# benfred/implicit

Hardware: AMD Instinct MI355X
Metric: ALS user+item updates/sec per iteration (factors=128); top-k recs/sec (higher is better)
Workload: dtype f32; 1 GPU; BASELINE configs[2]: last.fm-360K-shaped synthetic CSR, ALS CG cg_steps=3; users=358868, items=292385, nnz=17308340, factors=128, solver=cg, cg_steps=3

## Files before the change

implicit_amd/csrc/als_cg_q.hip:

```cpp
#include <type_traits>

#include "als_qtile.h"
#include "common.h"

namespace imp {

template <typename T>
void launch_team_fused(const imp_csr *C, int f, int width, int first, int count, T *X, const T *Y, const float *A0, int cg_steps,
                       const char *name);
template <typename T>
void launch_group_fused(const imp_csr *C, int f, int first, int count, T *X, const T *Y, const float *A0, int cg_steps, const char *name);
template <typename ST>
void launch_team_tile64(const imp_csr *C, int f, int width, int first, int count, ST *X, const ST *Y, const float *A0, int cg_steps,
                        const char *name);

template <typename T>
void launch_team_chain(const imp_csr *C, int f, const int (&first)[3], const int (&count)[3], T *X, const T *Y, const float *A0, int cg_steps,
                       const char *name);

template <int F, typename T> static void run_classes_q(const imp_csr *C, T *X, const T *Y, const float *A0, int cg_steps) {
  const int32_t *b = C->bin_start;
  constexpr bool kHalf = std::is_same<T, __half>::value;
  auto team = [&](int width32, int lo, int hi, const char *name) {
    if constexpr (kHalf) launch_team_tile64<T>(C, F, width32 / 2, lo, hi - lo, X, Y, A0, cg_steps, name);
    else launch_team_fused<T>(C, F, width32, lo, hi - lo, X, Y, A0, cg_steps, name);
  };
  team(16, b[1], b[2], "als_cg_team16_rows");
  if (F == 128 && !kHalf && !prof_unfiltered()) {
    const int first[3] = {b[2], b[3], b[4]}, count[3] = {b[3] - b[2], b[4] - b[3], b[5] - b[4]};
    launch_team_chain<T>(C, F, first, count, X, Y, A0, cg_steps, "als_cg_team_chain_rows");
  } else {
    team(8, b[2], b[3], "als_cg_team8_rows");
    team(4, b[3], b[4], "als_cg_team4_rows");
    team(2, b[4], b[5], "als_cg_team2_rows");
  }
  if constexpr (F == 64) launch_team_fused<T>(C, F, 1, b[5], b[7] - b[5], X, Y, A0, cg_steps, "als_cg_short_rows");
  else launch_group_fused<T>(C, F, b[5], b[7] - b[5], X, Y, A0, cg_steps, "als_cg_short_rows");
}

template <typename T> void least_squares_cg_q(const imp_csr *C, T *X, const T *Y, const float *A0, int f, int cg_steps) {
  if (f == 128) run_classes_q<128, T>(C, X, Y, A0, cg_steps);
  else if (f == 64) run_classes_q<64, T>(C, X, Y, A0, cg_steps);
  else throw std::invalid_argument("least_squares_cg_q: f must be 64 or 128");
}
template void least_squares_cg_q<float>(const imp_csr *, float *, const float *, const float *, int, int);
template void least_squares_cg_q<__half>(const imp_csr *, __half *, const __half *, const float *, int, int);

}
```

implicit_amd/csrc/als_cg_qf.hip:

```cpp
#include <type_traits>

#include <algorithm>

#include "als_qf_common.h"
#include "common.h"

namespace imp {

template <typename ST> struct Tile32 {
  typedef f32x2 elem;
  static constexpr int T = 32;
  static constexpr bool ROLL = std::is_same<ST, float>::value;
  static __device__ __forceinline__ void fetch(const int32_t *indices, const float *data, int lane, int k0, int end, int &col, float &c) {
    fetch_entries(indices, data, lane, k0, end, col, c);
  }
  template <int H> static __device__ __forceinline__ void gather(elem (&yq)[H], const ST *p) {
#pragma unroll
    for (int h = 0; h < H; h += 2) {
      const float4 v = load4(p + 32 * h);
      yq[h] = f32x2{v.x, v.y}, yq[h + 1] = f32x2{v.z, v.w};
    }
  }
  template <int H> static __device__ __forceinline__ float dot(const elem (&yq)[H], const f32x2 (&ve)[H]) {
    f32x2 s = yq[0] * ve[0];
// ... 156 lines not shown
  auto axpy = [&](int q, float w) { Tile::template axpy<H>(y[q], w, ae); };
  static_for<4>([&](auto Pc) {
    constexpr int P = decltype(Pc)::value;
    if (8 * P < cnt) {
      const float cm1_0 = cwg[8 * P];
      float cm1_1 = 0.f, cp_0 = 0.f, cp_1 = 0.f;
      if constexpr (!LAST) cm1_1 = cwg[8 * P + 4];
      if constexpr (FIRST) cp_0 = cwg[32 + 8 * P], cp_1 = cwg[32 + 8 * P + 4];
      const float u = reduce_pair(partial(2 * P), partial(2 * P + 1));
      if constexpr (LAST) {
        s8 = fmaf(cm1_0 * u, u, s8);
      } else {
        const float w0 = FIRST ? fmaf(-cm1_0, row_bcast_from<0>(u), cp_0) : cm1_0 * row_bcast_from<0>(u);
        const float w1 = FIRST ? fmaf(-cm1_1, row_bcast_from<8>(u), cp_1) : cm1_1 * row_bcast_from<8>(u);
        axpy(2 * P, w0);
        axpy(2 * P + 1, w1);
      }
    }
    if constexpr (ROLL) {
      if (8 * P < cnt_nx) gather_pair<Tile, F, P>(y, cw, col_nx, c_nx, cnt_nx, Y, lane);
    }
  });
  if constexpr (LAST) {
    return 0.125f * s8;
  } else {
    float aes[FE];
#pragma unroll
    for (int h = 0; h < H; ++h) aes[2 * h] = ae[h].x, aes[2 * h + 1] = ae[h].y;
    reduce_expanded<F>(aes, acc);
    return 0.f;
  }
}

template <int F, typename ST>
__global__ __launch_bounds__(1024) void als_cg_qfgroup_kernel(const int32_t *__restrict__ order, int first, int count,
                                                              const int32_t *__restrict__ indptr,
                                                              const int32_t *__restrict__ indices,
                                                              const float *__restrict__ data, ST *__restrict__ X,
                                                              const ST *__restrict__ Y, const float *__restrict__ A0, int cg_steps) {
  using Cfg = QFGroupCfg<F>;
  constexpr int FC = F / 64, FE = F / 16, LD = Cfg::LD;
  constexpr bool ROLL = Tile32<ST>::ROLL;
  extern __shared__ __attribute__((aligned(16))) float smem[];
  constexpr int LDB = Cfg::LDB;
  __bf16 *A0b = reinterpret_cast<__bf16 *>(smem);
  __bf16 *Pb = A0b + (size_t)3 * F * LDB;
  float *Ps = reinterpret_cast<float *>(Pb + (size_t)3 * 16 * LDB);
  float *Outs = Ps + 16 * LD;
  float *cws = Outs + (size_t)Cfg::KH * 16 * LD;
  const int lane = threadIdx.x & 63;
  const int wave = __builtin_amdgcn_readfirstlane(threadIdx.x >> 6);
  for (int e = threadIdx.x; e < F * F; e += 1024) {
    int r = e / F, c = e - r * F;
    __bf16 h, m, l;
    split_bf16(A0[e], h, m, l);
    A0b[r * LDB + c] = h, A0b[(size_t)F * LDB + r * LDB + c] = m, A0b[(size_t)2 * F * LDB + r * LDB + c] = l;
  }
  __syncthreads();
  float *prow = Ps + (size_t)wave * LD;
  float *cw = cws + (size_t)wave * 64;
  const unsigned cf = (unsigned)QL<F>::cfactor(lane, 0);

  auto publish = [&](const float (&vec)[FC], bool valid) {
    if constexpr (FC == 2) *reinterpret_cast<float2 *>(prow + cf) = valid ? make_float2(vec[0], vec[1]) : make_float2(0.f, 0.f);
    else prow[cf] = valid ? vec[0] : 0.f;
    bf16x2 t[3];
#pragma unroll
    for (int c = 0; c < 2; ++c) {
      __bf16 h, m, l;
      split_bf16(valid ? vec[c] : 0.f, h, m, l);
      t[0][c] = h, t[1][c] = m, t[2][c] = l;
    }
#pragma unroll
    for (int k = 0; k < 3; ++k) *reinterpret_cast<bf16x2 *>(Pb + (size_t)k * 16 * LDB + (size_t)wave * LDB + cf) = t[k];
    __syncthreads();
  };
  auto product = [&]() {
    const int ti = wave % Cfg::NT, kh = wave / Cfg::NT;
    const int ln = opaque(lane);
    const int i = ln & 15, kq = ln >> 4;
    f32x4 acc = {0.f, 0.f, 0.f, 0.f};
    static_assert(Cfg::KB * 16 == 64, "three-term product: 64 k per wave");
#pragma unroll
    for (int b = 0; b < 2; ++b) {
      const int k0 = kh * 64 + 32 * b + 8 * kq;
      const __bf16 *ar = A0b + (size_t)(16 * ti + i) * LDB + k0, *pr = Pb + (size_t)i * LDB + k0;
      const bf16x8 ah = *reinterpret_cast<const bf16x8 *>(ar), am = *reinterpret_cast<const bf16x8 *>(ar + (size_t)F * LDB),
                   al = *reinterpret_cast<const bf16x8 *>(ar + (size_t)2 * F * LDB);
      const bf16x8 ph = *reinterpret_cast<const bf16x8 *>(pr), pm = *reinterpret_cast<const bf16x8 *>(pr + (size_t)16 * LDB),
                   pl = *reinterpret_cast<const bf16x8 *>(pr + (size_t)2 * 16 * LDB);
      acc = __builtin_amdgcn_mfma_f32_16x16x32_bf16(al, ph, acc, 0, 0, 0);
      acc = __builtin_amdgcn_mfma_f32_16x16x32_bf16(ah, pl, acc, 0, 0, 0);
      acc = __builtin_amdgcn_mfma_f32_16x16x32_bf16(am, pm, acc, 0, 0, 0);
      acc = __builtin_amdgcn_mfma_f32_16x16x32_bf16(am, ph, acc, 0, 0, 0);
      acc = __builtin_amdgcn_mfma_f32_16x16x32_bf16(ah, pm, acc, 0, 0, 0);
      acc = __builtin_amdgcn_mfma_f32_16x16x32_bf16(ah, ph, acc, 0, 0, 0);
    }
    *reinterpret_cast<float4 *>(Outs + (kh * 16 + i) * LD + 16 * ti + 4 * kq) = make_float4(acc[0], acc[1], acc[2], acc[3]);
  };
  auto collect = [&](float (&out)[FC]) {
#pragma unroll
    for (int c = 0; c < FC; ++c) out[c] = 0.f;
#pragma unroll
    for (int h = 0; h < Cfg::KH; ++h) {
      const float *o = Outs + (h * 16 + wave) * LD + cf;
      if constexpr (FC == 2) {
        const float2 t = *reinterpret_cast<const float2 *>(o);
        out[0] += t.x, out[1] += t.y;
      } else {
        out[0] += o[0];
      }
    }
  };
  const bool product_first = ((wave >> 2) & 1) == 0;

  const int groups = (count + 15) / 16, g_step = gridDim.x;
  auto row_id = [&](int g) { return order[first + min(g * 16 + wave, count - 1)]; };
  auto row_valid = [&](int g) { return g < groups && g * 16 + wave < count; };
  int id0 = row_id(blockIdx.x), id1 = row_id(blockIdx.x + g_step), id2 = row_id(blockIdx.x + 2 * g_step), id3 = row_id(blockIdx.x + 3 * g_step);
  int b0 = indptr[id0], e0 = indptr[id0 + 1], b1 = indptr[id1], e1 = indptr[id1 + 1], b2 = indptr[id2], e2 = indptr[id2 + 1];
  int ent_col, ent_cnt = row_valid(blockIdx.x) ? e0 - b0 : 0;
  float ent_c;
  fetch_entries(indices, data, opaque(lane), b0, max(e0, b0 + 1), ent_col, ent_c);
  bool tile_ready = false;
  int cnt = 0;
  f32x2 y[8][FE / 2];
  float x[FC];
  auto kill = [](float (&v)[FC]) {
#pragma unroll
    for (int cc = 0; cc < FC; ++cc) v[cc] = 0.f;
  };
  kill(x);
  for (int g = blockIdx.x; g < groups; g += g_step) {
    const bool valid = row_valid(g);
    ST *xrow = X + (size_t)id0 * F;
    if (!tile_ready) {
      cnt = ent_cnt;
      ent_col = opaque(ent_col);
      ent_c = __int_as_float(opaque(__float_as_int(ent_c)));
      static_for<4>([&](auto Pc) {
        constexpr int P = decltype(Pc)::value;
        if (8 * P < cnt) gather_pair<Tile32<ST>, F, P>(y, cw, ent_col, ent_c, cnt, Y, lane);
      });
      ent_cnt = row_valid(g + g_step) ? e1 - b1 : 0;
      fetch_entries(indices, data, opaque(lane), b1, max(e1, b1 + 1), ent_col, ent_c);
      load_compact<F>(xrow, opaque(lane), x);
    }
    float xc[FC], r[FC], p[FC], Ap[FC], sp[FC];
#pragma unroll
    for (int cc = 0; cc < FC; ++cc) xc[cc] = x[cc];
    publish(xc, valid);
    if (!product_first) tile_pass<F, true, false, false, ST>(y, cw, cnt, prow, sp, lane, 0, ent_col, ent_c, Y);
    product();
    if (product_first) tile_pass<F, true, false, false, ST>(y, cw, cnt, prow, sp, lane, 0, ent_col, ent_c, Y);
    __syncthreads();
    collect(Ap);
#pragma unroll
    for (int cc = 0; cc < FC; ++cc) p[cc] = r[cc] = sp[cc] - Ap[cc];
    float rsold = dot_compact<F>(r, r);
    bool active = valid && rsold >= 1e-20f;
    const bool store = active;
    for (int it = 0; it + 1 < cg_steps; ++it) {
      publish(p, active);
      if (active && !product_first) tile_pass<F, false, false, false, ST>(y, cw, cnt, prow, sp, lane, 0, ent_col, ent_c, Y);
      product();
      if (active && product_first) tile_pass<F, false, false, false, ST>(y, cw, cnt, prow, sp, lane, 0, ent_col, ent_c, Y);
      __syncthreads();
      collect(Ap);
      if (active) {
#pragma unroll
        for (int cc = 0; cc < FC; ++cc) Ap[cc] += sp[cc];
        const float alpha = rsold * __builtin_amdgcn_rcpf(dot_compact<F>(p, Ap));
#pragma unroll
        for (int cc = 0; cc < FC; ++cc) {
          xc[cc] = fmaf(alpha, p[cc], xc[cc]);
          r[cc] = fmaf(-alpha, Ap[cc], r[cc]);
        }
        const float rsnew = dot_compact<F>(r, r);
        if (rsnew < 1e-20f) {
          active = false;
        } else {
          const float beta = rsnew * __builtin_amdgcn_rcpf(rsold);
#pragma unroll
          for (int cc = 0; cc < FC; ++cc) p[cc] = fmaf(beta, p[cc], r[cc]);
          rsold = rsnew;
        }
      }
    }
    bool rolled = false;
    if (cg_steps > 0) {
      publish(p, active);
      float tile_pAp = 0.f;
      auto last_tiles = [&]() {
        if constexpr (ROLL) tile_pAp = tile_pass<F, false, true, true, ST>(y, cw, cnt, prow, sp, lane, ent_cnt, ent_col, ent_c, Y);
        else tile_pAp = tile_pass<F, false, true, false, ST>(y, cw, cnt, prow, sp, lane, 0, ent_col, ent_c, Y);
      };
      if (active && !product_first) last_tiles();
      product();
      if (active && product_first) last_tiles();
      __syncthreads();
      collect(Ap);
      if (active) {
        if constexpr (ROLL) {
          cnt = ent_cnt;
          ent_cnt = row_valid(g + 2 * g_step) ? e2 - b2 : 0;
          fetch_entries(indices, data, opaque(lane), b2, max(e2, b2 + 1), ent_col, ent_c);
          load_compact<F>(X + (size_t)id1 * F, opaque(lane), x);
          rolled = true;
        } else {
          kill(x);
        }
        const float alpha = rsold * __builtin_amdgcn_rcpf(wave_allsum(dot_local<FC>(p, Ap) + tile_pAp));
#pragma unroll
        for (int cc = 0; cc < FC; ++cc) xc[cc] = fmaf(alpha, p[cc], xc[cc]);
      } else {
        kill(x);
      }
    } else {
      kill(x);
    }
    if (store) store_compact<F>(xrow, opaque(lane), xc);
    tile_ready = rolled;
    id0 = id1, id1 = id2, id2 = id3, id3 = row_id(g + 4 * g_step);
    b0 = b1, e0 = e1, b1 = b2, e1 = e2, b2 = indptr[id2], e2 = indptr[id2 + 1];
  }
}

template <typename T>
static void launch_qfgroup(const imp_csr *C, int first, int count, T *X, const T *Y, const float *A0, int cg_steps, const char *name) {
  if (count <= 0) return;
  constexpr int F = 128;
  const size_t lds = QFGroupCfg<F>::lds_bytes;
  auto kern = als_cg_qfgroup_kernel<F, T>;
  IMP_CHECK_HIP(hipFuncSetAttribute(reinterpret_cast<const void *>(kern), hipFuncAttributeMaxDynamicSharedMemorySize, (int)lds));
  int grid = std::min((count + 15) / 16, ctx().num_cus * std::max(2, ctx().oversub));
  IMP_PROF(name);
  kern<<<grid, 1024, lds, stream()>>>(C->order.data(), first, count, C->indptr.data(), C->indices.data(), C->data.data(), X, Y, A0,
                                      cg_steps);
  IMP_CHECK_HIP(hipGetLastError());
}

template <typename T>
void launch_group_fused(const imp_csr *C, int f, int first, int count, T *X, const T *Y, const float *A0, int cg_steps, const char *name) {
  if (f == 128) launch_qfgroup<T>(C, first, count, X, Y, A0, cg_steps, name);
  else throw std::invalid_argument("launch_group_fused: f must be 128 (f = 64 short rows run on independent wavefronts)");
}
template void launch_group_fused<float>(const imp_csr *, int, int, int, float *, const float *, const float *, int, const char *);
template void launch_group_fused<__half>(const imp_csr *, int, int, int, __half *, const __half *, const float *, int, const char *);

template <typename T>
void launch_team_fused(const imp_csr *C, int f, int width, int first, int count, T *X, const T *Y, const float *A0, int cg_steps,
                       const char *name) {
  if constexpr (std::is_same<T, __half>::value) {
    if (f != 64 || width != 1) throw std::invalid_argument("launch_team_fused: float16 storage takes the f = 64 short rows only");
    launch_qfteam<64, 1, 512, T>(C, first, count, X, Y, A0, cg_steps, name);
  } else {
    auto run = [&](auto Fc) {
      constexpr int F = decltype(Fc)::value;
      switch (width) {
        case 16: launch_qfteam<F, 16, 1024, T>(C, first, count, X, Y, A0, cg_steps, name); break;
        case 8: launch_qfteam<F, 8, 512, T>(C, first, count, X, Y, A0, cg_steps, name); break;
        case 4: launch_qfteam<F, 4, 512, T>(C, first, count, X, Y, A0, cg_steps, name); break;
        case 2: launch_qfteam<F, 2, 512, T>(C, first, count, X, Y, A0, cg_steps, name); break;
        case 1:
          if constexpr (F == 64) launch_qfteam<F, 1, 512, T>(C, first, count, X, Y, A0, cg_steps, name);
          else throw std::invalid_argument("launch_team_fused: one wave per row needs f = 64");
          break;
        default: throw std::invalid_argument("launch_team_fused: team width");
      }
    };
    if (f == 128) run(idx_t<128>{});
    else if (f == 64) run(idx_t<64>{});
    else throw std::invalid_argument("launch_team_fused: f must be 64 or 128");
// ... 8 lines not shown
```

implicit_amd/csrc/common.h:

```cpp
#ifndef IMPLICIT_AMD_CSRC_COMMON_H_
#define IMPLICIT_AMD_CSRC_COMMON_H_

#include <hip/hip_runtime.h>

#include <climits>
#include <cstdint>
#include <cstdio>
#include <memory>
#include <mutex>
#include <optional>
#include <stdexcept>
#include <string>
#include <vector>

#include "../../include/implicit_hip.h"
#include "csr_schedule.h"
#include "team_tickets.h"

namespace imp {

struct out_of_range_error : std::runtime_error {
  using std::runtime_error::runtime_error;
};

// ... 122 lines not shown
    const char *a = static_cast<const char *>(dst), *b = static_cast<const char *>(y_src);
    return b && a < b + y_rows * (size_t)y_f * sizeof(float) && b < a + bytes;
  }
  void release() {
    x = {}, y = {}, gram = {};
    forget_y();
  }
};

struct Context {
  int device = 0;
  hipStream_t stream = nullptr;
  int num_cus = 256;
  int oversub = 1;
  bool deferred = false;
  hipStream_t occupy_stream = nullptr;
  std::recursive_mutex mutex;
  std::mutex small_mutex;
  std::vector<void *> small_free[24];
  void *pin_stage = nullptr;
  size_t pin_stage_bytes = 0;
  hipEvent_t pin_stage_ev = nullptr;
  DeviceArray<float> gram_ws;
  DeviceArray<float> long_ws;
  PaddedSystem pad;
  DeviceArray<double> loss_buf;
  DeviceArray<unsigned long long> chol_failed;
  DeviceArray<float> barrier_word;
  unsigned long long *fixup_total = nullptr;
  DeviceArray<float> w256_ws;
  DeviceArray<unsigned> nm_fix_rows;
  DeviceArray<unsigned> chain_counters;
  ChainTickets chain_tickets;
  DeviceArray<int> nm_ticket;
  DeviceArray<unsigned long long> bpr_stats;
  DeviceArray<float> lmf_ws;
  DeviceArray<double> knn_acc;
  DeviceArray<int32_t> knn_touched;
  int knn_cols = -1;
};
inline hipStream_t stream() { return ctx().stream; }
void note_device_write(const void *dst, size_t bytes);
struct DerivedCache {
  const void *src = nullptr;
  size_t bytes = 0;
};
void register_derived_cache(DerivedCache *c);
void unregister_derived_cache(DerivedCache *c);

}

struct imp_matrix {
  size_t rows = 0, cols = 0, itemsize = 4;
  void *data = nullptr;
  std::shared_ptr<imp::Storage> storage;
  size_t bytes() const { return rows * cols * itemsize; }
  float *f32() const {
    if (itemsize != 4) throw std::runtime_error("can't cast Matrix to float*");
    return reinterpret_cast<float *>(data);
  }
};

struct imp_intvector {
  imp::DeviceArray<int32_t> v;
  size_t size = 0;
};
// ... 76 lines not shown
```

implicit_amd/csrc/containers.hip:

```cpp
#include <hip/hip_fp16.h>

#include <algorithm>
#include <cstring>
#include <map>
#include <mutex>
#include <thread>

#include "common.h"

namespace imp {

static thread_local std::string g_last_error;
void set_last_error(const std::string &msg) { g_last_error = msg; }

static std::mutex g_ctx_mutex;
static auto &g_contexts = *new std::map<int, std::unique_ptr<Context>>;

Context &ctx() {
  int dev = 0;
  IMP_CHECK_HIP(hipGetDevice(&dev));
  std::lock_guard<std::mutex> lock(g_ctx_mutex);
  auto it = g_contexts.find(dev);
  if (it == g_contexts.end()) {
    auto c = std::make_unique<Context>();
// ... 503 lines not shown
    std::copy(p.seg_row.begin(), p.seg_row.end(), seg_row);
    std::copy(p.seg_begin.begin(), p.seg_begin.end(), seg_begin);
    std::copy(p.seg_end.begin(), p.seg_end.end(), seg_end);
    std::copy(p.seg_exec.begin(), p.seg_exec.end(), seg_exec);
    std::copy(p.xcd_start, p.xcd_start + 9, xcd_start);
    const int32_t fields[8] = {p.n_long, p.n_seg, p.striped, s.n_chol_long, s.nm_segment, s.nm_multi_rows, s.nm_multi_segs, 0};
    std::copy(fields, fields + 8, info);
  });
}

int imp_host_chain_tickets(uint32_t *next, const int32_t *count, int32_t workgroups, const int32_t *teams_per_workgroup, uint32_t *base,
                           uint32_t *draws) {
  return guarded_host([&] {
    constexpr int NC = ChainTickets::kClasses, NQ = ChainTickets::kQueues;
    ChainTickets t;
    int32_t c[NC], n[NC];
    uint32_t b[NC][NQ];
    if (workgroups <= 0) throw std::invalid_argument("host_chain_tickets: the grid holds at least one workgroup");
    for (int k = 0; k < NC; ++k) {
      if (count[k] < 0 || count[k] >= ChainTickets::kMaxCount || teams_per_workgroup[k] <= 0)
        throw std::invalid_argument("host_chain_tickets: a class holds 0 .. 2^30 - 1 rows and a workgroup at least one team");
      c[k] = count[k], n[k] = teams_per_workgroup[k];
      for (int q = 0; q < NQ; ++q) t.next[k][q] = next[k * NQ + q];
    }
    t.launch(c, workgroups, n, b);
    for (int k = 0; k < NC; ++k)
      for (int q = 0; q < NQ; ++q) {
        draws[k * NQ + q] = t.next[k][q] - next[k * NQ + q];
        next[k * NQ + q] = t.next[k][q], base[k * NQ + q] = b[k][q];
      }
  });
}

int imp_matrix_create(size_t rows, size_t cols, const void *host_data, size_t itemsize, imp_matrix **out) {
  return guarded([&] {
    imp_matrix *m = new_matrix(rows, cols, itemsize, host_data == nullptr);
    std::unique_ptr<imp_matrix> guard(m);
    if (host_data && m->bytes()) {
      IMP_CHECK_HIP(hipMemcpyAsync(m->data, host_data, m->bytes(), hipMemcpyHostToDevice, stream()));
    }
    sync();
    *out = guard.release();
  });
}

int imp_matrix_wrap_device(size_t rows, size_t cols, void *device_ptr, size_t itemsize, imp_matrix **out) {
  return guarded([&] {
    if (itemsize != 4 && itemsize != 2) throw std::invalid_argument("invalid itemsize for Matrix (must be 2 or 4)");
    auto m = std::make_unique<imp_matrix>();
    m->rows = rows;
    m->cols = cols;
    m->itemsize = itemsize;
    m->storage = std::make_shared<Storage>(device_ptr);
    m->data = device_ptr;
    *out = m.release();
  });
}

int imp_matrix_row(const imp_matrix *src, size_t rowid, imp_matrix **out) {
  return guarded([&] {
    if (rowid >= src->rows) throw std::invalid_argument("row index out of bounds for matrix");
    auto m = std::make_unique<imp_matrix>(*src);
    m->rows = 1;
    m->data = reinterpret_cast<char *>(src->data) + rowid * src->cols * src->itemsize;
    *out = m.release();
  });
// ... 374 lines not shown
```

implicit_amd/csrc/team_tickets.h:

```cpp
#ifndef IMPLICIT_AMD_CSRC_TEAM_TICKETS_H_
#define IMPLICIT_AMD_CSRC_TEAM_TICKETS_H_

#include <algorithm>
#include <cstdint>

namespace imp {

struct ChainTickets {
  static constexpr int kClasses = 3;
  static constexpr int kQueues = 8;
  static constexpr int kCounterStride = 64;
  static constexpr int32_t kMaxCount = 1 << 30;
  uint32_t next[kClasses][kQueues] = {};

  static int32_t queue_rows(int32_t count, int q) { return count > q ? (count - q + kQueues - 1) / kQueues : 0; }
  static int32_t queue_workgroups(int32_t workgroups, int q) { return queue_rows(workgroups, q); }
  static uint32_t draws(int32_t count, int32_t teams) {
    if (count <= 0 || teams <= 0) return 0u;
    const int64_t n = teams, c = count;
    const int64_t inside = std::max<int64_t>(0, c - 4 * n);
    const int64_t past = std::min<int64_t>(n, std::max<int64_t>(0, c - 3 * n));
    return (uint32_t)(inside + past);
  }
  void launch(const int32_t (&count)[kClasses], int32_t workgroups, const int32_t (&teams_per_workgroup)[kClasses],
              uint32_t (&base)[kClasses][kQueues]) {
    for (int c = 0; c < kClasses; ++c)
      for (int q = 0; q < kQueues; ++q) {
        base[c][q] = next[c][q];
        next[c][q] += draws(queue_rows(count[c], q), queue_workgroups(workgroups, q) * teams_per_workgroup[c]);
      }
  }
};

}

#endif
```

implicit_amd/gpu/_hip.py:

```python
import ctypes
import os

_HERE = os.path.dirname(os.path.abspath(__file__))
from .. import _libpath

LIB_PATH = _libpath.OVERRIDE or os.path.join(os.path.dirname(_HERE), "libimplicit_hip.so")

c_void_pp = ctypes.POINTER(ctypes.c_void_p)
c_i32_p = ctypes.POINTER(ctypes.c_int32)
c_f32_p = ctypes.POINTER(ctypes.c_float)

IMP_OK, IMP_INVALID_ARGUMENT, IMP_OUT_OF_RANGE, IMP_RUNTIME_ERROR = 0, 1, 2, 3

_SIGNATURES = {
    "imp_get_device_count": [ctypes.POINTER(ctypes.c_int)],
    "imp_set_device": [ctypes.c_int],
    "imp_get_device": [ctypes.POINTER(ctypes.c_int)],
    "imp_set_oversubscribe": [ctypes.c_int],
    "imp_get_oversubscribe": [ctypes.POINTER(ctypes.c_int)],
    "imp_set_deferred_sync": [ctypes.c_int],
    "imp_debug_occupy": [ctypes.c_int, ctypes.c_int],
    "imp_debug_core_clock": [ctypes.c_int, ctypes.POINTER(ctypes.c_double)],
    "imp_device_synchronize": [],
    "imp_solver_fixup_rows": [ctypes.POINTER(ctypes.c_ulonglong), ctypes.c_int],
    "imp_mem_get_info": [ctypes.POINTER(ctypes.c_size_t), ctypes.POINTER(ctypes.c_size_t)],
    "imp_release_workspaces": [],
    "imp_host_csr_transpose": [ctypes.c_int32, ctypes.c_int32, ctypes.c_int64, ctypes.c_void_p, ctypes.c_void_p, ctypes.c_void_p,
                               ctypes.c_void_p, ctypes.c_void_p, ctypes.c_void_p, ctypes.c_int],
    "imp_host_csr_plan": [ctypes.c_int32, ctypes.c_int32, ctypes.c_void_p, ctypes.c_void_p, ctypes.c_int32, ctypes.c_int32,
                          ctypes.c_int32, ctypes.c_int32, ctypes.c_int, ctypes.c_void_p, ctypes.c_void_p, ctypes.c_void_p,
                          ctypes.c_int64, ctypes.c_void_p, ctypes.c_void_p, ctypes.c_void_p, ctypes.c_void_p, ctypes.c_void_p,
                          ctypes.c_void_p],
    "imp_host_chain_tickets": [ctypes.c_void_p, ctypes.c_void_p, ctypes.c_int32, ctypes.c_void_p, ctypes.c_void_p, ctypes.c_void_p],
    "imp_matrix_create": [ctypes.c_size_t, ctypes.c_size_t, ctypes.c_void_p, ctypes.c_size_t, c_void_pp],
    "imp_matrix_wrap_device": [ctypes.c_size_t, ctypes.c_size_t, ctypes.c_void_p, ctypes.c_size_t, c_void_pp],
    "imp_matrix_row": [ctypes.c_void_p, ctypes.c_size_t, c_void_pp],
    "imp_matrix_slice": [ctypes.c_void_p, ctypes.c_size_t, ctypes.c_size_t, c_void_pp],
    "imp_matrix_gather": [ctypes.c_void_p, ctypes.c_void_p, c_void_pp],
    "imp_matrix_resize": [ctypes.c_void_p, ctypes.c_size_t, ctypes.c_size_t],
    "imp_matrix_assign_rows": [ctypes.c_void_p, ctypes.c_void_p, ctypes.c_void_p],
    "imp_matrix_astype": [ctypes.c_void_p, ctypes.c_size_t, c_void_pp],
    "imp_matrix_calculate_norms": [ctypes.c_void_p, c_void_pp],
    "imp_matrix_to_host": [ctypes.c_void_p, ctypes.c_void_p],
    "imp_matrix_from_host": [ctypes.c_void_p, ctypes.c_void_p],
    "imp_matrix_copy_rows": [ctypes.c_void_p, ctypes.c_size_t, ctypes.c_void_p, ctypes.c_size_t, ctypes.c_size_t],
    "imp_matrix_shape": [ctypes.c_void_p, ctypes.POINTER(ctypes.c_size_t), ctypes.POINTER(ctypes.c_size_t),
                         ctypes.POINTER(ctypes.c_size_t)],
    "imp_matrix_device_ptr": [ctypes.c_void_p, c_void_pp],
    "imp_matrix_destroy": [ctypes.c_void_p],
    "imp_intvector_create": [ctypes.c_void_p, ctypes.c_size_t, c_void_pp],
    "imp_intvector_destroy": [ctypes.c_void_p],
    "imp_csr_create": [ctypes.c_int32, ctypes.c_int32, ctypes.c_int64, ctypes.c_void_p, ctypes.c_void_p,
                       ctypes.c_void_p, c_void_pp],
    "imp_csr_create64": [ctypes.c_int32, ctypes.c_int32, ctypes.c_int64, ctypes.c_void_p, ctypes.c_void_p,
                         ctypes.c_void_p, c_void_pp],
    "imp_csr_shape": [ctypes.c_void_p, c_i32_p, c_i32_p, ctypes.POINTER(ctypes.c_int64)],
    "imp_csr_destroy": [ctypes.c_void_p],
    "imp_coo_create": [ctypes.c_int32, ctypes.c_int32, ctypes.c_int64, ctypes.c_void_p, ctypes.c_void_p,
                       ctypes.c_void_p, c_void_pp],
    "imp_coo_create_from_csr_pattern": [ctypes.c_int32, ctypes.c_int32, ctypes.c_void_p, ctypes.c_int, ctypes.c_void_p,
                                        ctypes.POINTER(ctypes.c_void_p)],
    "imp_coo_destroy": [ctypes.c_void_p],
    "imp_solver_create": [c_void_pp],
    "imp_solver_destroy": [ctypes.c_void_p],
    "imp_solver_calculate_yty": [ctypes.c_void_p, ctypes.c_void_p, ctypes.c_void_p, ctypes.c_float],
    "imp_solver_least_squares": [ctypes.c_void_p, ctypes.c_void_p, ctypes.c_void_p, ctypes.c_void_p,
# ... 103 lines not shown
```

implicit_amd/utils.py:

```python
import time
import warnings

import numpy as np
import scipy.sparse


class ParameterWarning(Warning):
    """Raised (as a warning) when an input had to be converted (implicit/utils.py:155-156)."""


def check_csr(user_items):
    if isinstance(user_items, scipy.sparse.csr_matrix):
        return user_items
    kind = type(user_items).__name__
    t0 = time.time()
    converted = user_items.tocsr()
    warnings.warn(
        f"Method expects CSR input, and was passed {kind} instead. "
        f"Converting to CSR took {time.time() - t0} seconds",
        ParameterWarning,
    )
    return converted


# ... 115 lines not shown
    from .gpu._hip import check, lib

    rows, cols = m.shape
    indptr = np.ascontiguousarray(m.indptr, dtype=np.int32)
    indices = np.ascontiguousarray(m.indices, dtype=np.int32)
    capacity = max(int(indptr[-1]), 0) if rows else 0
    out = {"order": np.empty(rows, np.int32), "bin_start": np.empty(9, np.int32), "row_seg": np.empty(rows + 1, np.int32)}
    segs = {k: np.empty(capacity, np.int32) for k in ("seg_row", "seg_begin", "seg_end", "seg_exec")}
    out["xcd_start"] = np.empty(9, np.int32)
    info = np.zeros(8, np.int32)
    check(lib().imp_host_csr_plan(rows, cols, indptr.ctypes.data, indices.ctypes.data, segment, stripe, nm_segment, num_cus, which,
                                  out["order"].ctypes.data, out["bin_start"].ctypes.data, out["row_seg"].ctypes.data, capacity,
                                  *(segs[k].ctypes.data for k in ("seg_row", "seg_begin", "seg_end", "seg_exec")),
                                  out["xcd_start"].ctypes.data, info.ctypes.data))
    names = ("n_long", "n_seg", "striped", "n_chol_long", "nm_segment", "nm_multi_rows", "nm_multi_segs")
    out.update({k: int(v) for k, v in zip(names, info)})
    out["striped"] = bool(out["striped"])
    out["row_seg"] = out["row_seg"][:out["n_long"] + 1]
    out.update({k: v[:out["n_seg"]] for k, v in segs.items()})
    return out


def chain_tickets(state, counts, workgroups, teams_per_workgroup=(1, 2, 4)):
    from .gpu._hip import check, lib

    assert state.dtype == np.uint32 and state.shape == (3, 8) and state.flags.c_contiguous
    counts = np.ascontiguousarray(counts, dtype=np.int32)
    teams = np.ascontiguousarray(teams_per_workgroup, dtype=np.int32)
    assert counts.shape == teams.shape == (3,)
    base, draws = np.empty((3, 8), np.uint32), np.empty((3, 8), np.uint32)
    check(lib().imp_host_chain_tickets(state.ctypes.data, counts.ctypes.data, int(workgroups), teams.ctypes.data, base.ctypes.data,
                                       draws.ctypes.data))
    return base, draws
```

include/implicit_hip.h:

```cpp
#ifndef IMPLICIT_HIP_H_
#define IMPLICIT_HIP_H_

#include <stddef.h>
#include <stdint.h>

#ifdef __cplusplus
extern "C" {
#endif

typedef enum {
  IMP_OK = 0,
  IMP_INVALID_ARGUMENT = 1,
  IMP_OUT_OF_RANGE = 2,
  IMP_RUNTIME_ERROR = 3
} imp_status;

typedef struct imp_matrix imp_matrix;
typedef struct imp_intvector imp_intvector;
typedef struct imp_csr imp_csr;
typedef struct imp_coo imp_coo;
typedef struct imp_solver imp_solver;
typedef struct imp_knn imp_knn;
typedef struct imp_random imp_random;
typedef struct imp_comm imp_comm;

const char *imp_last_error(void);
int imp_get_device_count(int *count);
int imp_set_device(int device);
int imp_get_device(int *device);
int imp_set_oversubscribe(int factor);
int imp_get_oversubscribe(int *factor);
int imp_set_deferred_sync(int on);
int imp_debug_occupy(int workgroups, int microseconds);
int imp_debug_core_clock(int microseconds, double *mhz);
int imp_device_synchronize(void);
int imp_solver_fixup_rows(unsigned long long *count, int reset);
int imp_mem_get_info(size_t *free_bytes, size_t *total_bytes);
int imp_release_workspaces(void);
const char *imp_version(void);

int imp_host_csr_transpose(int32_t rows, int32_t cols, int64_t nonzeros, const int32_t *indptr, const int32_t *indices,
                           const float *data, int32_t *t_indptr, int32_t *t_indices, float *t_data, int threads);

int imp_host_csr_plan(int32_t rows, int32_t cols, const int32_t *indptr, const int32_t *indices, int32_t segment, int32_t stripe,
                      int32_t nm_segment, int32_t num_cus, int which, int32_t *order, int32_t *bin_start, int32_t *row_seg,
                      int64_t seg_capacity, int32_t *seg_row, int32_t *seg_begin, int32_t *seg_end, int32_t *seg_exec,
                      int32_t *xcd_start, int32_t *info);

int imp_host_chain_tickets(uint32_t *next, const int32_t *count, int32_t workgroups, const int32_t *teams_per_workgroup, uint32_t *base,
                           uint32_t *draws);

int imp_matrix_create(size_t rows, size_t cols, const void *host_data, size_t itemsize, imp_matrix **out);
int imp_matrix_wrap_device(size_t rows, size_t cols, void *device_ptr, size_t itemsize, imp_matrix **out);
int imp_matrix_row(const imp_matrix *m, size_t rowid, imp_matrix **out);
int imp_matrix_slice(const imp_matrix *m, size_t start, size_t end, imp_matrix **out);
int imp_matrix_gather(const imp_matrix *m, const imp_intvector *rowids, imp_matrix **out);
int imp_matrix_resize(imp_matrix *m, size_t rows, size_t cols);
int imp_matrix_assign_rows(imp_matrix *m, const imp_intvector *rowids, const imp_matrix *other);
int imp_matrix_astype(const imp_matrix *m, size_t itemsize, imp_matrix **out);
int imp_matrix_calculate_norms(const imp_matrix *m, imp_matrix **out);
int imp_matrix_to_host(const imp_matrix *m, void *host_out);
int imp_matrix_from_host(imp_matrix *m, const void *host_in);
int imp_matrix_copy_rows(imp_matrix *dst, size_t dst_row, const imp_matrix *src, size_t src_row, size_t rows);
int imp_matrix_shape(const imp_matrix *m, size_t *rows, size_t *cols, size_t *itemsize);
int imp_matrix_device_ptr(const imp_matrix *m, void **ptr);
int imp_matrix_destroy(imp_matrix *m);

int imp_intvector_create(const int32_t *host_data, size_t size, imp_intvector **out);
int imp_intvector_destroy(imp_intvector *v);
int imp_csr_create(int32_t rows, int32_t cols, int64_t nonzeros, const int32_t *indptr,
                   const int32_t *indices, const float *data, imp_csr **out);
int imp_csr_create64(int32_t rows, int32_t cols, int64_t nonzeros, const int64_t *indptr,
                     const int32_t *indices, const float *data, imp_csr **out);
int imp_csr_shape(const imp_csr *m, int32_t *rows, int32_t *cols, int64_t *nonzeros);
int imp_csr_destroy(imp_csr *m);
int imp_coo_create(int32_t rows, int32_t cols, int64_t nonzeros, const int32_t *row,
                   const int32_t *col, const float *data, imp_coo **out);
int imp_coo_create_from_csr_pattern(int32_t rows, int32_t cols, const void *indptr, int indptr_is_64,
                                    const int32_t *indices, imp_coo **out);
int imp_coo_destroy(imp_coo *m);

int imp_solver_create(imp_solver **out);
int imp_solver_destroy(imp_solver *s);
// ... 84 lines not shown
```

Before: 171.5 million updates/s.

## Fuse team16 and short-row classes into one ticketed wide-chain kernel

For f=128 fp32, the separate team16 launch and the short-row group launch are merged into one persistent kernel. Each workgroup first works through the longest rows as team16, then stages the Gramian and processes the short-row groups. Work is handed out through per-queue atomic ticket counters, which replaces the static grid-stride assignment. The goal is to cut launch count, shorten tail idle time between classes and balance load dynamically, at the cost of atomic traffic and higher LDS sizing (the max of both classes), which may lower occupancy.

```diff
diff --git a/implicit_amd/csrc/als_cg_q.hip b/implicit_amd/csrc/als_cg_q.hip
--- a/implicit_amd/csrc/als_cg_q.hip
+++ b/implicit_amd/csrc/als_cg_q.hip
@@ -17,6 +17,9 @@
 template <typename T>
 void launch_team_chain(const imp_csr *C, int f, const int (&first)[3], const int (&count)[3], T *X, const T *Y, const float *A0, int cg_steps,
                        const char *name);
+template <typename T>
+void launch_wide_chain(const imp_csr *C, int f, const int (&first)[2], const int (&count)[2], T *X, const T *Y, const float *A0, int cg_steps,
+                       const char *name);
 
 template <int F, typename T> static void run_classes_q(const imp_csr *C, T *X, const T *Y, const float *A0, int cg_steps) {
   const int32_t *b = C->bin_start;
@@ -25,15 +28,17 @@
     if constexpr (kHalf) launch_team_tile64<T>(C, F, width32 / 2, lo, hi - lo, X, Y, A0, cg_steps, name);
     else launch_team_fused<T>(C, F, width32, lo, hi - lo, X, Y, A0, cg_steps, name);
   };
-  team(16, b[1], b[2], "als_cg_team16_rows");
   if (F == 128 && !kHalf && !prof_unfiltered()) {
     const int first[3] = {b[2], b[3], b[4]}, count[3] = {b[3] - b[2], b[4] - b[3], b[5] - b[4]};
     launch_team_chain<T>(C, F, first, count, X, Y, A0, cg_steps, "als_cg_team_chain_rows");
-  } else {
-    team(8, b[2], b[3], "als_cg_team8_rows");
-    team(4, b[3], b[4], "als_cg_team4_rows");
-    team(2, b[4], b[5], "als_cg_team2_rows");
+    const int wide_first[2] = {b[1], b[5]}, wide_count[2] = {b[2] - b[1], b[7] - b[5]};
+    launch_wide_chain<T>(C, F, wide_first, wide_count, X, Y, A0, cg_steps, "als_cg_wide_chain_rows");
+    return;
   }
+  team(16, b[1], b[2], "als_cg_team16_rows");
+  team(8, b[2], b[3], "als_cg_team8_rows");
+  team(4, b[3], b[4], "als_cg_team4_rows");
+  team(2, b[4], b[5], "als_cg_team2_rows");
   if constexpr (F == 64) launch_team_fused<T>(C, F, 1, b[5], b[7] - b[5], X, Y, A0, cg_steps, "als_cg_short_rows");
   else launch_group_fused<T>(C, F, b[5], b[7] - b[5], X, Y, A0, cg_steps, "als_cg_short_rows");
 }
diff --git a/implicit_amd/csrc/als_cg_qf.hip b/implicit_amd/csrc/als_cg_qf.hip
--- a/implicit_amd/csrc/als_cg_qf.hip
+++ b/implicit_amd/csrc/als_cg_qf.hip
@@ -212,12 +212,23 @@
   }
 }
 
-template <int F, typename ST>
-__global__ __launch_bounds__(1024) void als_cg_qfgroup_kernel(const int32_t *__restrict__ order, int first, int count,
-                                                              const int32_t *__restrict__ indptr,
-                                                              const int32_t *__restrict__ indices,
-                                                              const float *__restrict__ data, ST *__restrict__ X,
-                                                              const ST *__restrict__ Y, const float *__restrict__ A0, int cg_steps) {
+template <int F> __device__ __forceinline__ void group_stage_gramian(const float *__restrict__ A0) {
+  extern __shared__ __attribute__((aligned(16))) float smem[];
+  constexpr int LDB = QFGroupCfg<F>::LDB;
+  __bf16 *A0b = reinterpret_cast<__bf16 *>(smem);
+  for (int e = threadIdx.x; e < F * F; e += 1024) {
+    int r = e / F, c = e - r * F;
+    __bf16 h, m, l;
+    split_bf16(A0[e], h, m, l);
+    A0b[r * LDB + c] = h, A0b[(size_t)F * LDB + r * LDB + c] = m, A0b[(size_t)2 * F * LDB + r * LDB + c] = l;
+  }
+  __syncthreads();
+}
+
+template <int F, typename ST, bool TICKETS = false>
+__device__ __forceinline__ void group_rows(const int32_t *__restrict__ order, int first, int count, const int32_t *__restrict__ indptr,
+                                           const int32_t *__restrict__ indices, const float *__restrict__ data, ST *__restrict__ X,
+                                           const ST *__restrict__ Y, int cg_steps, unsigned *counter = nullptr, unsigned base = 0u) {
   using Cfg = QFGroupCfg<F>;
   constexpr int FC = F / 64, FE = F / 16, LD = Cfg::LD;
   constexpr bool ROLL = Tile32<ST>::ROLL;
@@ -230,13 +241,6 @@
   float *cws = Outs + (size_t)Cfg::KH * 16 * LD;
   const int lane = threadIdx.x & 63;
   const int wave = __builtin_amdgcn_readfirstlane(threadIdx.x >> 6);
-  for (int e = threadIdx.x; e < F * F; e += 1024) {
-    int r = e / F, c = e - r * F;
-    __bf16 h, m, l;
-    split_bf16(A0[e], h, m, l);
-    A0b[r * LDB + c] = h, A0b[(size_t)F * LDB + r * LDB + c] = m, A0b[(size_t)2 * F * LDB + r * LDB + c] = l;
-  }
-  __syncthreads();
   float *prow = Ps + (size_t)wave * LD;
   float *cw = cws + (size_t)wave * 64;
   const unsigned cf = (unsigned)QL<F>::cfactor(lane, 0);
@@ -294,12 +298,28 @@
   };
   const bool product_first = ((wave >> 2) & 1) == 0;
 
-  const int groups = (count + 15) / 16, g_step = gridDim.x;
-  auto row_id = [&](int g) { return order[first + min(g * 16 + wave, count - 1)]; };
-  auto row_valid = [&](int g) { return g < groups && g * 16 + wave < count; };
-  int id0 = row_id(blockIdx.x), id1 = row_id(blockIdx.x + g_step), id2 = row_id(blockIdx.x + 2 * g_step), id3 = row_id(blockIdx.x + 3 * g_step);
+  const int queue = TICKETS ? (int)(blockIdx.x % kTicketQueues) : 0;
+  const int all_groups = (count + 15) / 16;
+  const int groups = TICKETS ? (all_groups - queue + kTicketQueues - 1) / kTicketQueues : all_groups;
+  const int g_step = TICKETS ? (int)((gridDim.x - queue + kTicketQueues - 1) / kTicketQueues) : (int)gridDim.x;
+  const int g_first = TICKETS ? (int)(blockIdx.x / kTicketQueues) : (int)blockIdx.x;
+  auto row_of = [&](int g) { return (TICKETS ? kTicketQueues * g + queue : g) * 16 + wave; };
+  auto row_id = [&](int g) { return order[first + min(row_of(g), count - 1)]; };
+  auto row_valid = [&](int g) { return g < groups && row_of(g) < count; };
+  int t1 = g_first + g_step, t2 = g_first + 2 * g_step, t3 = g_first + 3 * g_step;
+  unsigned drawn = 0u;
+  unsigned *ticket_word = reinterpret_cast<unsigned *>(cws + 16 * 64);
+  auto draw = [&]() {
+    if (lane == 0) asm volatile("global_atomic_add %0, %1, %2, off sc0" : "=v"(drawn) : "v"(counter), "v"(1u) : "memory");
+  };
+  auto take_draw = [&]() {
+    asm volatile("s_waitcnt vmcnt(0)" : "+v"(drawn)::"memory");
+    const unsigned t = min((unsigned)__builtin_amdgcn_readfirstlane(drawn) - base + 4u * (unsigned)g_step, (unsigned)groups);
+    if (lane == 0) *ticket_word = t;
+  };
+  int id0 = row_id(g_first), id1 = row_id(t1), id2 = row_id(t2), id3 = row_id(t3);
   int b0 = indptr[id0], e0 = indptr[id0 + 1], b1 = indptr[id1], e1 = indptr[id1 + 1], b2 = indptr[id2], e2 = indptr[id2 + 1];
-  int ent_col, ent_cnt = row_valid(blockIdx.x) ? e0 - b0 : 0;
+  int ent_col, ent_cnt = row_valid(g_first) ? e0 - b0 : 0;
   float ent_c;
   fetch_entries(indices, data, opaque(lane), b0, max(e0, b0 + 1), ent_col, ent_c);
   bool tile_ready = false;
@@ -311,8 +331,9 @@
     for (int cc = 0; cc < FC; ++cc) v[cc] = 0.f;
   };
   kill(x);
-  for (int g = blockIdx.x; g < groups; g += g_step) {
+  for (int g = g_first; g < groups;) {
     const bool valid = row_valid(g);
+    int t_new = t3 + g_step;
     ST *xrow = X + (size_t)id0 * F;
     if (!tile_ready) {
       cnt = ent_cnt;
@@ -322,7 +343,7 @@
         constexpr int P = decltype(Pc)::value;
         if (8 * P < cnt) gather_pair<Tile32<ST>, F, P>(y, cw, ent_col, ent_c, cnt, Y, lane);
       });
-      ent_cnt = row_valid(g + g_step) ? e1 - b1 : 0;
+      ent_cnt = row_valid(t1) ? e1 - b1 : 0;
       fetch_entries(indices, data, opaque(lane), b1, max(e1, b1 + 1), ent_col, ent_c);
       load_compact<F>(xrow, opaque(lane), x);
     }
@@ -330,10 +351,20 @@
 #pragma unroll
     for (int cc = 0; cc < FC; ++cc) xc[cc] = x[cc];
     publish(xc, valid);
+    const bool drawing = TICKETS && t3 < groups;
+    if constexpr (TICKETS) {
+      if (drawing && wave == 0) draw();
+    }
     if (!product_first) tile_pass<F, true, false, false, ST>(y, cw, cnt, prow, sp, lane, 0, ent_col, ent_c, Y);
     product();
     if (product_first) tile_pass<F, true, false, false, ST>(y, cw, cnt, prow, sp, lane, 0, ent_col, ent_c, Y);
+    if constexpr (TICKETS) {
+      if (drawing && wave == 0) take_draw();
+    }
     __syncthreads();
+    if constexpr (TICKETS) {
+      t_new = drawing ? (int)__builtin_amdgcn_readfirstlane(*reinterpret_cast<volatile unsigned *>(ticket_word)) : groups;
+    }
     collect(Ap);
 #pragma unroll
     for (int cc = 0; cc < FC; ++cc) p[cc] = r[cc] = sp[cc] - Ap[cc];
@@ -383,7 +414,7 @@
       if (active) {
         if constexpr (ROLL) {
           cnt = ent_cnt;
-          ent_cnt = row_valid(g + 2 * g_step) ? e2 - b2 : 0;
+          ent_cnt = row_valid(t2) ? e2 - b2 : 0;
           fetch_entries(indices, data, opaque(lane), b2, max(e2, b2 + 1), ent_col, ent_c);
           load_compact<F>(X + (size_t)id1 * F, opaque(lane), x);
           rolled = true;
@@ -401,9 +432,20 @@
     }
     if (store) store_compact<F>(xrow, opaque(lane), xc);
     tile_ready = rolled;
-    id0 = id1, id1 = id2, id2 = id3, id3 = row_id(g + 4 * g_step);
+    g = t1, t1 = t2, t2 = t3, t3 = t_new;
+    id0 = id1, id1 = id2, id2 = id3, id3 = row_id(t3);
     b0 = b1, e0 = e1, b1 = b2, e1 = e2, b2 = indptr[id2], e2 = indptr[id2 + 1];
   }
+}
+
+template <int F, typename ST>
+__global__ __launch_bounds__(1024) void als_cg_qfgroup_kernel(const int32_t *__restrict__ order, int first, int count,
+                                                              const int32_t *__restrict__ indptr,
+                                                              const int32_t *__restrict__ indices,
+                                                              const float *__restrict__ data, ST *__restrict__ X,
+                                                              const ST *__restrict__ Y, const float *__restrict__ A0, int cg_steps) {
+  group_stage_gramian<F>(A0);
+  group_rows<F, ST>(order, first, count, indptr, indices, data, X, Y, cg_steps);
 }
 
 template <typename T>
@@ -419,6 +461,86 @@
                                       cg_steps);
   IMP_CHECK_HIP(hipGetLastError());
 }
+
+#ifndef IMP_WIDE_FORM
+#define IMP_WIDE_FORM 0
+#endif
+struct WideClassArgs {
+  int first[WideTickets::kClasses], count[WideTickets::kClasses];
+  unsigned base[WideTickets::kClasses][WideTickets::kQueues];
+};
+static_assert(WideTickets::kQueues == kTicketQueues && WideTickets::kGroupRows == 16, "queues and groups of the ticketed classes");
+template <int F> constexpr size_t wide_chain_lds_bytes() {
+  return std::max(team_lds_bytes<F, 16, 1024, 32>(), QFGroupCfg<F>::lds_bytes + 16);
+}
+template <int F, typename ST, bool SHORT_TICKETS>
+__global__ __launch_bounds__(1024) void als_cg_qfwide_chain_kernel(const int32_t *__restrict__ order, WideClassArgs cls,
+                                                                   unsigned *__restrict__ counters,
+                                                                   const int32_t *__restrict__ indptr,
+                                                                   const int32_t *__restrict__ indices,
+                                                                   const float *__restrict__ data, ST *__restrict__ X,
+                                                                   const ST *__restrict__ Y, const float *__restrict__ A0,
+                                                                   int cg_steps) {
+  const unsigned queue = blockIdx.x % kTicketQueues;
+  if (cls.count[0] > 0)
+    team_rows<Tile32<ST>, F, 16, 1024, true, true>(order, cls.first[0], cls.count[0], indptr, indices, data, X, Y, A0, cg_steps,
+                                                   counters + queue * WideTickets::kCounterStride, cls.base[0][queue]);
+  if (cls.count[1] > 0) {
+    if (cls.count[0] > 0) __syncthreads();
+    group_stage_gramian<F>(A0);
+    group_rows<F, ST, SHORT_TICKETS>(order, cls.first[1], cls.count[1], indptr, indices, data, X, Y, cg_steps,
+                                     counters + (kTicketQueues + queue) * WideTickets::kCounterStride, cls.base[1][queue]);
+  }
+}
+
+template <typename T>
+void launch_wide_chain(const imp_csr *C, int f, const int (&first)[2], const int (&count)[2], T *X, const T *Y, const float *A0, int cg_steps,
+                       const char *name) {
+  if constexpr (std::is_same<T, float>::value) {
+    if (f != 128) throw std::invalid_argument("launch_wide_chain: f must be 128");
+    constexpr int F = 128;
+    constexpr bool kShortTickets = IMP_WIDE_FORM != 1;
+    if (count[0] <= 0 && count[1] <= 0) return;
+    const size_t lds = wide_chain_lds_bytes<F>();
+    auto kern = als_cg_qfwide_chain_kernel<F, T, kShortTickets>;
+    static const int per_cu = [&] {
+      int n = 0;
+      IMP_CHECK_HIP(hipFuncSetAttribute(reinterpret_cast<const void *>(kern), hipFuncAttributeMaxDynamicSharedMemorySize, (int)lds));
+      IMP_CHECK_HIP(hipOccupancyMaxActiveBlocksPerMultiprocessor(&n, reinterpret_cast<const void *>(kern), 1024, lds));
+      if (n < 1) throw std::runtime_error("launch_wide_chain: the kernel does not fit a compute unit");
+      return n;
+    }();
+    IMP_CHECK_HIP(hipFuncSetAttribute(reinterpret_cast<const void *>(kern), hipFuncAttributeMaxDynamicSharedMemorySize, (int)lds));
+    const int grid = std::max(ctx().num_cus * per_cu, WideTickets::kQueues);
+    for (int c = 0; c < 2; ++c)
+      if (count[c] >= WideTickets::kMaxCount) throw std::invalid_argument("launch_wide_chain: too many rows in a class");
+    Context &cx = ctx();
+    if (!cx.wide_counters.data())
+      cx.wide_counters.alloc((size_t)WideTickets::kClasses * WideTickets::kQueues * WideTickets::kCounterStride, true);
+    auto run = [&](bool on0, bool on1) {
+      WideClassArgs cls;
+      const int32_t rows[2] = {on0 ? std::max(count[0], 0) : 0, on1 ? std::max(count[1], 0) : 0};
+      if (rows[0] == 0 && rows[1] == 0) return;
+      for (int c = 0; c < 2; ++c) cls.first[c] = first[c], cls.count[c] = rows[c];
+      WideTickets after = cx.wide_tickets;
+      const int32_t ticketed[2] = {rows[0], kShortTickets ? rows[1] : 0};
+      after.launch_rows(ticketed, grid, cls.base);
+      kern<<<grid, 1024, lds, stream()>>>(C->order.data(), cls, cx.wide_counters.data(), C->indptr.data(), C->indices.data(),
+                                         C->data.data(), X, Y, A0, cg_steps);
+      IMP_CHECK_HIP(hipGetLastError());
+      cx.wide_tickets = after;
+    };
+    IMP_PROF(name);
+    if (IMP_WIDE_FORM == 2) run(true, false), run(false, true);
+    else run(true, true);
+  } else {
+    throw std::invalid_argument("launch_wide_chain: fp32 storage only");
+  }
+}
+template void launch_wide_chain<float>(const imp_csr *, int, const int (&)[2], const int (&)[2], float *, const float *, const float *, int,
+                                       const char *);
+template void launch_wide_chain<__half>(const imp_csr *, int, const int (&)[2], const int (&)[2], __half *, const __half *, const float *,
+                                        int, const char *);
 
 template <typename T>
 void launch_group_fused(const imp_csr *C, int f, int first, int count, T *X, const T *Y, const float *A0, int cg_steps, const char *name) {
diff --git a/implicit_amd/csrc/common.h b/implicit_amd/csrc/common.h
--- a/implicit_amd/csrc/common.h
+++ b/implicit_amd/csrc/common.h
@@ -178,6 +178,8 @@
   DeviceArray<unsigned> nm_fix_rows;
   DeviceArray<unsigned> chain_counters;
   ChainTickets chain_tickets;
+  DeviceArray<unsigned> wide_counters;
+  WideTickets wide_tickets;
   DeviceArray<int> nm_ticket;
   DeviceArray<unsigned long long> bpr_stats;
   DeviceArray<float> lmf_ws;
diff --git a/implicit_amd/csrc/containers.hip b/implicit_amd/csrc/containers.hip
--- a/implicit_amd/csrc/containers.hip
+++ b/implicit_amd/csrc/containers.hip
@@ -559,6 +559,27 @@
   });
 }
 
+int imp_host_wide_tickets(uint32_t *next, const int32_t *rows, int32_t workgroups, uint32_t *base, uint32_t *draws) {
+  return guarded_host([&] {
+    constexpr int NC = WideTickets::kClasses, NQ = WideTickets::kQueues;
+    WideTickets t;
+    uint32_t b[NC][NQ];
+    if (workgroups <= 0) throw std::invalid_argument("host_wide_tickets: the grid holds at least one workgroup");
+    for (int k = 0; k < NC; ++k) {
+      if (rows[k] < 0 || rows[k] >= WideTickets::kMaxCount)
+        throw std::invalid_argument("host_wide_tickets: a class holds 0 .. 2^30 - 1 rows");
+      for (int q = 0; q < NQ; ++q) t.next[k][q] = next[k * NQ + q];
+    }
+    const int32_t r[NC] = {rows[0], rows[1]};
+    t.launch_rows(r, workgroups, b);
+    for (int k = 0; k < NC; ++k)
+      for (int q = 0; q < NQ; ++q) {
+        draws[k * NQ + q] = t.next[k][q] - next[k * NQ + q];
+        next[k * NQ + q] = t.next[k][q], base[k * NQ + q] = b[k][q];
+      }
+  });
+}
+
 int imp_matrix_create(size_t rows, size_t cols, const void *host_data, size_t itemsize, imp_matrix **out) {
   return guarded([&] {
     imp_matrix *m = new_matrix(rows, cols, itemsize, host_data == nullptr);
diff --git a/implicit_amd/csrc/team_tickets.h b/implicit_amd/csrc/team_tickets.h
--- a/implicit_amd/csrc/team_tickets.h
+++ b/implicit_amd/csrc/team_tickets.h
@@ -6,8 +6,8 @@
 
 namespace imp {
 
-struct ChainTickets {
-  static constexpr int kClasses = 3;
+template <int NC> struct TicketClasses {
+  static constexpr int kClasses = NC;
   static constexpr int kQueues = 8;
   static constexpr int kCounterStride = 64;
   static constexpr int32_t kMaxCount = 1 << 30;
@@ -32,6 +32,17 @@
   }
 };
 
+typedef TicketClasses<3> ChainTickets;
+
+struct WideTickets : TicketClasses<2> {
+  static constexpr int kGroupRows = 16;
+  static int32_t groups(int32_t rows) { return rows > 0 ? (rows + kGroupRows - 1) / kGroupRows : 0; }
+  void launch_rows(const int32_t (&rows)[2], int32_t workgroups, uint32_t (&base)[2][kQueues]) {
+    const int32_t units[2] = {rows[0], groups(rows[1])}, teams[2] = {1, 1};
+    launch(units, workgroups, teams, base);
+  }
+};
+
 }
 
 #endif
diff --git a/implicit_amd/gpu/_hip.py b/implicit_amd/gpu/_hip.py
--- a/implicit_amd/gpu/_hip.py
+++ b/implicit_amd/gpu/_hip.py
@@ -32,6 +32,7 @@
                           ctypes.c_int64, ctypes.c_void_p, ctypes.c_void_p, ctypes.c_void_p, ctypes.c_void_p, ctypes.c_void_p,
                           ctypes.c_void_p],
     "imp_host_chain_tickets": [ctypes.c_void_p, ctypes.c_void_p, ctypes.c_int32, ctypes.c_void_p, ctypes.c_void_p, ctypes.c_void_p],
+    "imp_host_wide_tickets": [ctypes.c_void_p, ctypes.c_void_p, ctypes.c_int32, ctypes.c_void_p, ctypes.c_void_p],
     "imp_matrix_create": [ctypes.c_size_t, ctypes.c_size_t, ctypes.c_void_p, ctypes.c_size_t, c_void_pp],
     "imp_matrix_wrap_device": [ctypes.c_size_t, ctypes.c_size_t, ctypes.c_void_p, ctypes.c_size_t, c_void_pp],
     "imp_matrix_row": [ctypes.c_void_p, ctypes.c_size_t, c_void_pp],
diff --git a/implicit_amd/utils.py b/implicit_amd/utils.py
--- a/implicit_amd/utils.py
+++ b/implicit_amd/utils.py
@@ -171,3 +171,14 @@
     check(lib().imp_host_chain_tickets(state.ctypes.data, counts.ctypes.data, int(workgroups), teams.ctypes.data, base.ctypes.data,
                                        draws.ctypes.data))
     return base, draws
+
+
+def wide_tickets(state, rows, workgroups):
+    from .gpu._hip import check, lib
+
+    assert state.dtype == np.uint32 and state.shape == (2, 8) and state.flags.c_contiguous
+    rows = np.ascontiguousarray(rows, dtype=np.int32)
+    assert rows.shape == (2,)
+    base, draws = np.empty((2, 8), np.uint32), np.empty((2, 8), np.uint32)
+    check(lib().imp_host_wide_tickets(state.ctypes.data, rows.ctypes.data, int(workgroups), base.ctypes.data, draws.ctypes.data))
+    return base, draws
diff --git a/include/implicit_hip.h b/include/implicit_hip.h
--- a/include/implicit_hip.h
+++ b/include/implicit_hip.h
@@ -49,6 +49,8 @@
 
 int imp_host_chain_tickets(uint32_t *next, const int32_t *count, int32_t workgroups, const int32_t *teams_per_workgroup, uint32_t *base,
                            uint32_t *draws);
+
+int imp_host_wide_tickets(uint32_t *next, const int32_t *rows, int32_t workgroups, uint32_t *base, uint32_t *draws);
 
 int imp_matrix_create(size_t rows, size_t cols, const void *host_data, size_t itemsize, imp_matrix **out);
 int imp_matrix_wrap_device(size_t rows, size_t cols, void *device_ptr, size_t itemsize, imp_matrix **out);
```

Result: faster. 175.4 million updates/s (median of 6 runs) (+2.3%).
